# aras-p/ToyPathTracer

Measured on AMD Instinct MI355X. Metric: Mray/s, higher is better.
Workload: dtype f32

## Files before the change

toypathtracer_amd/csrc/tpt_device.h:

```cpp
#pragma once
#include "tpt_trace.h"

#ifndef TPT_BLOCK
#define TPT_BLOCK 64
#endif
#define TPT_CHUNK_PIXELS 256

namespace tpt {

struct KernelArgs {
    SceneView scene;
    FrameConsts fc;
    f4* frameColour;
    int nLocalRows, stripeRows, stripeStride, stripeOffset;
    int tilesX;
    int numItems;
    int numChunks, chunkSize;
    int batchFrames, chunksPerFrame, framePlane;
    unsigned totalWaves;
    int laneCap;
    int noRefill;
    f4* stackBuf;
    int stackStride;
    int ldsStackLevels;
    f4* pathBuf;
    const unsigned* chunkOrder;
    unsigned* chunkCost;
    int chunkShift;
    unsigned* work;
    unsigned long long* rayCounter;
    int rayCounterStride;
    unsigned gen;
    int helperBase;
    int helperPct;
    int ldsGroupPairs;
    const CameraPOD* viewCams = nullptr;
    const f4* moveCentres = nullptr;
    f4* aovSums = nullptr;
    f4* aovAlbedo = nullptr;
    f4* aovNormalDepth = nullptr;
    f4* momentsOut = nullptr;
    int aovPlane = 0;
    const int32_t* sampleCounts = nullptr;
    const f4* keyCentres = nullptr;
    unsigned long long keyMask = 0;
    int keyCount = 0;
};

}

hipError_t tptLaunchTrace(const tpt::KernelArgs& a, int hs, int fold, bool ldsScene, int blocks, size_t lds, hipStream_t stream);
int tptTraceOccupancy(int hs, int fold, bool ldsScene, size_t lds);
hipError_t tptLaunchTraceQueue(const tpt::KernelArgs& a, bool ldsScene, int blocks, size_t lds, hipStream_t stream);
int tptQueueMatrixFilter();
int tptQueueGroupMatrixBounds();
hipError_t tptLaunchDisplay(const float* tile, unsigned char* rgba, int width, int height, hipStream_t stream);
__attribute__((weak)) hipError_t tptLaunchDenoise(const float* colour, const float* albedo, const float* normalDepth, float* out,
                                                  float* scratch, int width, int height, int iterations, float ic, float in, float id,
                                                  bool demodulate, hipStream_t stream);
__attribute__((weak)) hipError_t tptLaunchDenoiseVariance(const float* colour, const float* albedo, const float* normalDepth,
                                                          const float* moments, float* out, float* scratch, int width, int height,
                                                          int iterations, float samples, float sl2, float in, float id, bool demodulate,
                                                          hipStream_t stream);
__attribute__((weak)) hipError_t tptLaunchFramesAtrous(const float* colour, const float* albedo, const float* normalDepth,
                                                       const float* moments, float* out, float* scratch, int width, int height, int frames,
                                                       int iterations, float samples, float sl2, float in, float id, bool demodulate,
                                                       hipStream_t stream);
struct tptTemporalConsts {
    float o[3], ll[3], H[3], V[3];
    float po[3], pa[3], pw[3], pH[3], pV[3];
    float pf, phh, pvv;
    float maxHistory, depthTol, normalTol, coverageTol;
};
__attribute__((weak)) hipError_t tptLaunchTemporal(const float* colour, const float* albedo, const float* normalDepth, const float* moments,
                                                   const float* prevColour, const float* prevAlbedo, const float* prevNormalDepth,
                                                   const float* prevMoments, float* outColour, float* outAlbedo, float* outMoments,
                                                   float* outVariance, int width, int height, const tptTemporalConsts& k,
                                                   hipStream_t stream);
struct tptObjectPlaneConsts {
// ... 53 lines not shown
```

toypathtracer_amd/csrc/tpt_host_pipeline.cpp:

```cpp
#include "tpt_context.h"

using namespace tpt;
using namespace tpth;

namespace tpth {

struct FramePlan {
    KernelArgs a;
    bool rowSerial = false, queued = false, ldsScene = false, useOrder = false;
    size_t lds = 0;
    int occ = 0, threadsPerBlock = 0, blocks = 0;
    int nOverlap = 1;
    int nSlots = 1, slot = 0;
    int batch = 1;
    bool plainFrame = true;
    const char* entry = "tptDrawDevice";
};

int syncAllStreams();
int reserveSlotBuffers(int nSlots, size_t colourBytes, size_t stackBytes)
{
    const bool small = colourBytes * 4 <= g.colourCap && g.colourCap * (size_t)g.slotsReserved > (1ull << 30);
    g.smallStreak = small ? g.smallStreak + 1 : 0;
    const bool shrink = small && g.smallStreak >= 8 && g.pending.empty();
// ... 504 lines not shown
            }
            (void)hipGetLastError();
        }
        HIPCHK(hipStreamWaitEvent(ts, g.evResolve[slot], 0));
    }
    if ((rc = enqueueSceneUpload(ts))) return rc;
    if (aov && ts != g.stream) {
        if (clip) {
            const unsigned h = g.clipSeq & 1u;
            HIPCHK(hipEventRecord(g.evClip[h ^ 1u], g.stream));
            HIPCHK(hipStreamWaitEvent(ts, aov->continues ? g.evClip[h] : g.evClip[h ^ 1u], 0));
        } else {
            HIPCHK(hipEventRecord(g.evAov, g.stream));
            HIPCHK(hipStreamWaitEvent(ts, g.evAov, 0));
        }
    }
    if (clip) g.clipSeq++;
    if (viewCams || centres || keyCentres) {
        static_assert(2 * sizeof(f4) * kMaxBatch <= sizeof(CameraPOD) * kMaxBatch, "a batch's moving centres fit the slot's camera table");
        Context::ViewSlot& V = g.views[slot];
        const f4* behind = keyCentres ? keyCentres : centres;
        const size_t camBytes = sizeof(CameraPOD) * (size_t)batch, centreBytes = (keyCentres ? (size_t)TPT_Q_KEYS_MAX : 2) * sizeof(f4) * (size_t)batch;
        const size_t bytes = viewCams && behind ? kViewCamBytes + centreBytes : (viewCams ? camBytes : centreBytes);
        if (V.copyEnqueued) HIPCHK(hipEventSynchronize(V.evUploaded));
        if (viewCams) memcpy(V.stage, viewCams, camBytes);
        if (behind) memcpy(reinterpret_cast<char*>(V.stage) + (viewCams ? kViewCamBytes : 0), behind, centreBytes);
        HIPCHK(hipMemcpyAsync(V.dev, V.stage, bytes, hipMemcpyHostToDevice, ts));
        HIPCHK(hipEventRecord(V.evUploaded, ts));
        V.copyEnqueued = true;
    }
    if ((rc = enqueueChunkOrder(P, ts))) return rc;
    if (frameRays && frameRays != g.dRays) HIPCHK(hipMemsetAsync(frameRays, 0, sizeof(unsigned long long) * (size_t)(rayStride > 0 ? batch : 1), ts));
    const bool helpable = P.queued && pipelined && batch == 1 && !P.rowSerial && !table && !aov;
    a.helperBase = 0;
    a.helperPct = 0;
    a.gen = 0u;
    g.hrec[slot].valid = false;
    if (helpable) {
        if (++g.launchGen == 0u) g.launchGen = 1u;
        a.gen = g.launchGen;
        HIPCHK(hipEventRecord(g.evPre[slot], ts));
    }
    const bool timeIt = g.kernelTiming && g.ktUsed < g.ktStart.size();
    if (timeIt) HIPCHK(hipEventRecord(g.ktStart[g.ktUsed], ts));
    if (P.queued)
        HIPCHK(tptLaunchTraceQueue(a, P.ldsScene, P.blocks, P.lds, ts));
    else
        HIPCHK(tptLaunchTrace(a, g.hs, g.foldMode, P.ldsScene, P.blocks, P.lds, ts));
    seqGuard.launched = true;
    if (timeIt) {
        HIPCHK(hipEventRecord(g.ktStop[g.ktUsed], ts));
        g.ktUsed++;
    }
    if (pipelined) HIPCHK(hipEventRecord(g.evTrace[slot], ts));
    if (helpable) {
        Context::HelperRec& R = g.hrec[slot];
        R.a = a; R.ldsScene = P.ldsScene; R.blocks = P.blocks; R.maxBlocks = maxGridBlocks(P); R.lds = P.lds;
        R.helped = false; R.valid = true; R.ts = ts;
    }
    T.slot = slot;
    T.nPixels = a.nLocalRows * w;
    T.pipelined = pipelined;
    T.lerpFac = a.fc.lerpFac;
    T.colour = a.frameColour;
    T.moments = a.momentsOut;
    T.batch = batch;
// ... 617 lines not shown
```

toypathtracer_amd/csrc/tpt_kernels.hip:

```cpp
#include "../../include/tpt_hip.h"
#include "tpt_device.h"
#include "tpt_queue_layout.h"
#include "tpt_shard.h"

namespace tpt {

__device__ __forceinline__ unsigned waveReduceAdd(unsigned v)
{
#pragma unroll
    for (int off = 32; off > 0; off >>= 1) v += __shfl_down(v, off, 64);
    return v;
}

__device__ __forceinline__ void storeColour(const KernelArgs& a, const Lane& L)
{
    f3 c = lanePixelColour(L, a.fc);
    f4 v;
    v.x = c.x; v.y = c.y; v.z = c.z; v.w = 0.0f;
    a.frameColour[L.pix] = v;
}

__global__ void __launch_bounds__(256) tptResolveKernel(float* __restrict__ tile, const f4* __restrict__ colour, int nPixels, float lerpFac,
                                                        const unsigned long long* frameRays, unsigned long long* totalRays)
{
// ... 1501 lines not shown
                    cm2 &= sel == 2 ? keep : ~0ull;
                    cm3 &= sel == 3 ? keep : ~0ull;
                    list[pos] = ((unsigned)p << 16) | (unsigned)((pb0 + sel * 32) * 2 + k);
                    ++pos;
                }
                if (!parked) {
                    st[p] = mk4(u2f((uint32_t)id), hitT, o.x, o.y);
                    st[PATHS + p] = mk4(o.z, d.x, d.y, d.z);
                    parked = true;
                }
            }
            __builtin_amdgcn_wave_barrier();
            dealProcessList<PATHS>(sv, list, listCount, st, lane);
            __builtin_amdgcn_wave_barrier();
        }
    }
    if (parked) {
        const f4 k = st[p];
        id = (int)f2u(k.x);
        hitT = k.y;
    }
    outT = hitT;
    return id;
}
#endif

#ifndef TPT_Q_MIN_WAVES_PER_SIMD
#define TPT_Q_MIN_WAVES_PER_SIMD 4
#endif
#ifndef TPT_Q_MAX_VGPR
#define TPT_Q_MAX_VGPR 60
#endif
template <bool LDS_SCENE, bool BATCH, bool VIEWS = false, bool MOVING = false, bool AOV = false, bool MOMENTS = false, bool ADAPTIVE = false,
          bool CAMERAS = false, bool KEYS = false>
__device__ __forceinline__ void traceQueueBody(const KernelArgs& a)
{
    extern __shared__ __attribute__((aligned(16))) unsigned char smem[];
    static_assert(BATCH || !VIEWS, "views are frames of a batched launch");
    static_assert((BATCH || !MOVING) && !(VIEWS && MOVING), "animation frames are frames of a batched launch of their own");
    static_assert(!AOV || !BATCH || (MOVING && MOMENTS), "first-hit planes are made by single-frame launches, or beside the moments of an animated clip's frames");
    static_assert(!MOMENTS || AOV, "moments are summed beside the first-hit sums");
    static_assert(!ADAPTIVE || (MOMENTS && !BATCH), "a count per pixel belongs to a single frame with its moments");
    static_assert(!CAMERAS || (BATCH && MOVING && AOV && MOMENTS && !VIEWS && !ADAPTIVE), "a camera per frame belongs to the frames of a clip with their planes");
    static_assert(!KEYS || CAMERAS, "the caller's centres per frame belong to the frames of a clip with their cameras and planes");
    constexpr bool CAM_TABLE = VIEWS || CAMERAS;
    constexpr int kMovedPerFrame = KEYS ? TPT_Q_KEYS_MAX : 2;
    constexpr int kPaths = (LDS_SCENE ? TPT_Q_PATHS : TPT_Q_PATHS_GROUPED) - (CAM_TABLE ? TPT_Q_VIEW_PATHS : 0) -
                           (MOVING ? (KEYS ? TPT_Q_KEY_PATHS : TPT_Q_ANIM_PATHS) : 0);
    constexpr int kOffSt = LDS_SCENE ? TPT_Q_SPH_FIXED : 0;
    constexpr int kOffQ = kOffSt + TPT_Q_NF4 * kPaths * 16;
    constexpr int kOffCtl = kOffQ + Q_COUNT * TPT_Q_P * 2;
    constexpr int kOffDeal = kOffCtl + (((int)sizeof(QueueCtl) + 63) & ~63);
    constexpr int kDealBytes = (!LDS_SCENE && TPT_GROUP_DEAL) ? TPT_Q_WAVES * TPT_GROUP_DEAL_WAVE_BYTES : 0;
    constexpr int kOffFc = kOffDeal + kDealBytes;
    constexpr int kOffCams = kOffFc + (((int)sizeof(FrameConsts) + 15) & ~15);
    constexpr int kOffMoved = kOffCams + (CAM_TABLE ? TPT_Q_VIEW_CAM_BYTES : 0);
    constexpr int kOffScene = kOffMoved + (MOVING ? (KEYS ? TPT_Q_KEY_TABLE_BYTES : TPT_Q_ANIM_TABLE_BYTES) : 0);
    f4* st = reinterpret_cast<f4*>(smem + kOffSt);
    LdsRing q = (LdsRing)(smem + kOffQ);
    QueueCtl* ctl = reinterpret_cast<QueueCtl*>(smem + kOffCtl);
    FrameConsts* ldsFc = reinterpret_cast<FrameConsts*>(smem + kOffFc);
    CameraPOD* ldsCams = reinterpret_cast<CameraPOD*>(smem + kOffCams);
    f4* ldsMoved = reinterpret_cast<f4*>(smem + kOffMoved);
    const LdsMovedPtr movedLds = (LdsMovedPtr)ldsMoved;
    const int nPad = a.scene.nPairs * 2;
    const bool sphFixed = LDS_SCENE && nPad * 16 <= TPT_Q_SPH_FIXED;
    f4* ldsSphFixed = reinterpret_cast<f4*>(smem);
    f4* ldsSph = sphFixed ? ldsSphFixed : reinterpret_cast<f4*>(smem + kOffScene);
    int off = kOffScene + ((LDS_SCENE && !sphFixed) ? nPad * 16 : 0);
// ... 58 lines not shown
        for (int i = tid; i < a.batchFrames * (int)(sizeof(CameraPOD) / 4); i += TPT_Q_T)
            reinterpret_cast<uint32_t*>(ldsCams)[i] = reinterpret_cast<const uint32_t*>(a.viewCams)[i];
    if (MOVING)
        for (int i = tid; i < a.batchFrames * kMovedPerFrame; i += TPT_Q_T) ldsMoved[i] = KEYS ? a.keyCentres[i] : a.moveCentres[i];
    const uint64_t keyMask = KEYS ? (uint64_t)a.keyMask : 0ull;
    for (int i = tid; i < Q_COUNT * TPT_Q_P; i += TPT_Q_T) q[i] = (unsigned short)(i < kPaths ? i : 0xFFFF);
    if (tid < 8) {
        ctl->head[tid] = 0u;
        ctl->tail[tid] = tid == Q_FREE ? (unsigned)kPaths : 0u;
    }
    if (tid == 0) {
        ctl->poolTotal = 0u;
        ctl->globalExhausted = 0u;
    }
    if (BATCH && tid < 32) ctl->frameRays[tid] = 0u;
    __syncthreads();

    const FrameConsts& fc = a.fc;
    const unsigned long long laneBelow = (1ull << lane) - 1ull;
#if TPT_MATRIX_FILTER
    SceneView svM = sv;
    svM.sph4 = ldsSphFixed;
#endif
#if TPT_GROUP_DEAL
    LdsList dealList = (LdsList)(smem + kOffDeal + (tid >> 6) * TPT_GROUP_DEAL_WAVE_BYTES);
    unsigned* dealCount = reinterpret_cast<unsigned*>(smem + kOffDeal + (tid >> 6) * TPT_GROUP_DEAL_WAVE_BYTES + TPT_GROUP_DEAL_ENTRIES * 4);
    const bool groupDeal = !MOVING && !LDS_SCENE && sv.nGroups > 0 && sv.nGroups <= 65536;
#endif
    f4* colSum = st + 2 * kPaths;
    int chunkNext = 0, chunkEnd = 0;
    int chunkFrame = 0;
    bool noMoreChunks = false;
    unsigned myRays = 0;
#if defined(TPT_STATS)
    const unsigned long long qT0 = wall_clock64();
    unsigned qSteps = 0, qBatches = 0, qIdle = 0;
    unsigned long long qSec[5] = {0, 0, 0, 0, 0};
#endif

#if defined(TPT_STATS)
#define TPT_TSTAMP(v)                      \
    __builtin_amdgcn_sched_barrier(0);     \
    __builtin_amdgcn_s_waitcnt(0);         \
    const unsigned long long v = __builtin_amdgcn_s_memtime(); \
    __builtin_amdgcn_sched_barrier(0)
#if TPT_STATS < 2
#define TPT_TADD(slot, a, b) do { if (lane == 0) atomicAdd(&g_tptStats[slot], (b) - (a)); } while (0)
#else
#define TPT_TADD(slot, a, b) do { qSec[(slot) == 64 + 24 ? 4 : ((slot) & 3)] += (b) - (a); } while (0)
#endif
#else
#define TPT_TSTAMP(v) do { } while (0)
#define TPT_TADD(slot, a, b) do { } while (0)
#endif
    for (;;) {
        TPT_TSTAMP(tsTop);
        unsigned myAvail = 0, myHead = 0, myTail = 0;
        if (lane < Q_COUNT) {
            myTail = __hip_atomic_load(&ctl->tail[lane], __ATOMIC_RELAXED, __HIP_MEMORY_SCOPE_WORKGROUP);
            myHead = __hip_atomic_load(&ctl->head[lane], __ATOMIC_RELAXED, __HIP_MEMORY_SCOPE_WORKGROUP);
            myAvail = myTail - myHead;
        }
        unsigned avail[Q_COUNT];
#pragma unroll
        for (int c = 0; c < Q_COUNT; ++c) avail[c] = (unsigned)__builtin_amdgcn_readlane((int)myAvail, c);
        const bool canStart = (chunkEnd > chunkNext) || !noMoreChunks;
// ... 55 lines not shown
        QStack stack;
        stack.l0 = (LdsF4Ptr)(st + 3 * kPaths + p);
        stack.spill = a.stackBuf + ((size_t)(blockIdx.x + (unsigned)a.helperBase) * TPT_Q_PATHS + p);
        stack.stride = a.stackStride;
        constexpr int kAovSums = MOMENTS ? 3 : 2;
        auto aovSum = [&]() { return a.aovSums + kAovSums * ((size_t)(blockIdx.x + (unsigned)a.helperBase) * TPT_Q_PATHS + p); };
        QLambert lam;
        lam.sdir = lam.nl = lam.albedo = lam.lightE = mk3(0, 0, 0);
        lam.cosAMax = 0.0f;
        int movedAt = 0;
        if (pick != Q_FREE && mine) {
            if (MOVING) movedAt = kMovedPerFrame * (int)(f2u(colSum[p].w) >> 26);
            const f4 r0 = st[0 * kPaths + p], r1 = st[1 * kPaths + p];
            ro = mk3(r0.x, r0.y, r0.z);
            rng = f2u(r0.w);
            rd = mk3(r1.x, r1.y, r1.z);
            const uint32_t w = f2u(r1.w);
            sample = (int)(w & 0x7ffu);
            depth = (int)((w >> 11) & 15u);
            doMatE = ((w >> 15) & 1u) != 0;
            recId = (w >> 16) == 0xffffu ? -1 : (int)(w >> 16);
        }

        if (pick == Q_FREE) {
            bool need = mine, got = false;
            int px = 0, py = 0, laneFrame = 0;
            [[maybe_unused]] uint32_t laneCount = 0u;
            for (;;) {
                const unsigned long long needMask = __ballot(need);
                if (needMask == 0ull) break;
                if (chunkNext >= chunkEnd) {
                    if (noMoreChunks) break;
                    int c = 0;
                    if (lane == 0) {
                        atomicAdd(&ctl->poolTotal, 64u);
                        c = (int)atomicAdd(&a.work[0], 1u);
                    }
                    c = __builtin_amdgcn_readfirstlane(c);
                    if (c >= a.numChunks) {
                        if (lane == 0) {
                            atomicSub(&ctl->poolTotal, 64u);
                            __hip_atomic_store(&ctl->globalExhausted, 1u, __ATOMIC_RELAXED, __HIP_MEMORY_SCOPE_WORKGROUP);
                        }
                        noMoreChunks = true;
                        break;
                    }
                    chunkFrame = 0;
                    if (BATCH) {
                        chunkFrame = c / a.chunksPerFrame;
                        c -= chunkFrame * a.chunksPerFrame;
                    }
                    chunkNext = c * a.chunkSize;
                    chunkEnd = chunkNext + a.chunkSize;
                    if (chunkEnd > a.numItems) chunkEnd = a.numItems;
                    if (lane == 0 && chunkEnd - chunkNext != 64) atomicSub(&ctl->poolTotal, (unsigned)(64 - (chunkEnd - chunkNext)));
                }
                const int rank = __popcll(needMask & laneBelow);
                const int want = __popcll(needMask);
                const int availPx = chunkEnd - chunkNext;
                const int take = want < availPx ? want : availPx;
                if (need && rank < take) {
                    int x, ly;
                    bool take1 = mapItem(a, chunkNext + rank, x, ly);
                    if (ADAPTIVE && take1) {
                        const int c = a.sampleCounts[(size_t)ly * fc.width + x];
                        laneCount = (uint32_t)(c < 0 ? 0 : (c > 2047 ? 2047 : c));
                        take1 = laneCount != 0u;
                    }
                    if (take1) {
                        px = x;
                        py = localRowToGlobal(a, ly);
                        laneFrame = chunkFrame;
                        got = true;
                        need = false;
                    }
                }
                chunkNext += take;
                if (lane == 0) atomicSub(&ctl->poolTotal, (unsigned)take);
            }
            if (got) {
                rng = pixelSeed(fc.seedMode, px, py, fc.frame + ((BATCH && !VIEWS) ? laneFrame : 0));
// ... 120 lines not shown
                        const f4 l0 = MOVING ? movedOrKeyedSphere<KEYS>(sv.lights[j * 2], lightId, movedLds + movedAt, keyMask) : sv.lights[j * 2];
                        d2 = qLightRay(l0, ro, rng, lam.cosAMax, (sv.flags & SCENE_LIGHT_R2_DIV_SAFE) != 0);
                    }
                }
#if TPT_MATRIX_FILTER
                uint64_t cand = 0ull;
                if (LDS_SCENE && useMatrix) cand = phase1MatrixH(ldsA, mxR1, sv.nSpheres, ro, d2);
#endif
#if TPT_GROUP_DEAL
                int dealId = -1;
                float dealT = TPT_MAX_T;
                if (!LDS_SCENE && groupDeal)
                    dealId = hitSpheresGroupedDeal<kPaths>(sv, go, ro, d2, dealT, dealList, dealCount, st, p, lane, ldsGpairs, a.ldsGroupPairs);
#endif
                if (go) {
                    TPT_STAT(ST_STEP);
                    float t;
                    int id;
#if TPT_GROUP_DEAL
                    if (!LDS_SCENE && groupDeal) {
                        id = dealId;
                        t = dealT;
                    } else
#endif
#if TPT_MATRIX_FILTER
                    if (LDS_SCENE && useMatrix)
                        id = hitSpheresCandidates<MOVING, KEYS>(svM, cand, ro, d2, TPT_MIN_T, TPT_MAX_T, t, movedLds + movedAt, keyMask);
                    else
#endif
                    if (MOVING)
                        id = hitSpheresTwoPhase<true, KEYS>(sv, ro, d2, TPT_MIN_T, TPT_MAX_T, t, movedLds + movedAt, keyMask);
                    else
                        id = hitSpheres<LDS_SCENE ? HS_TWO_PHASE : HS_TWO_PHASE_GROUPS>(sv, ro, d2, TPT_MIN_T, TPT_MAX_T, t);
                    if (BATCH) iterRays++; else myRays++;
                    if (shadow) {
                        if (id == lightId) qLightShade(l1, d2, lam);
                    } else {
                        hitId = id;
                        hitT = t;
                    }
                }
            }
            if (ray) {
                if (hitId < 0 || depth >= TPT_MAX_DEPTH)
                    cls = Q_END;
                else {
                    const int type = (int)f2u(sv.mats[hitId * 3].w);
                    cls = type == MAT_LAMBERT ? Q_LAMBERT : type == MAT_METAL ? Q_METAL : type == MAT_DIELECTRIC ? Q_DIEL : Q_END;
                }
                if (hitId >= 0) ro = ro + rd * hitT;
                if (AOV && depth == 0 && hitId >= 0) {
                    const f3 nrm = qNormal<MOVING, KEYS>(sv, hitId, ro, movedLds + movedAt, keyMask);
                    const f4 m0 = sv.mats[hitId * 3];
                    f4* sum = aovSum();
                    const f4 s0 = sum[0], s1 = sum[1];
                    sum[0] = mk4(s0.x + m0.x, s0.y + m0.y, s0.z + m0.z, s0.w + 1.0f);
                    sum[1] = mk4(s1.x + nrm.x, s1.y + nrm.y, s1.z + nrm.z, s1.w + hitT);
                }
                recId = hitId;
            }
        } else if (ray) {
            cls = Q_INT;
        }
        if (toEnd) cls = Q_END;
        if (ray || toEnd) {
            const uint32_t w = ((uint32_t)sample & 0x7ffu) | (((uint32_t)depth & 15u) << 11) | ((uint32_t)doMatE << 15) | (((uint32_t)recId & 0xffffu) << 16);
            st[0 * kPaths + p] = mk4(ro.x, ro.y, ro.z, u2f(rng));
            st[1 * kPaths + p] = mk4(rd.x, rd.y, rd.z, u2f(w));
        }
        if (toFree) cls = Q_FREE;
        if (BATCH && iterRays != 0u) {
            const unsigned fr = f2u(colSum[p].w) >> 26;
            const unsigned old = atomicAdd(&ctl->frameRays[fr], iterRays);
            if (__builtin_expect(old < 0x80000000u && old + iterRays >= 0x80000000u, 0)) {
                atomicSub(&ctl->frameRays[fr], 0x80000000u);
                atomicAdd(a.rayCounter + (size_t)fr * a.rayCounterStride, 0x80000000ull);
            }
        }
        TPT_TSTAMP(tsInt);
        TPT_TADD(64 + pick * 4 + 2, tsClass, tsInt);
        __builtin_amdgcn_fence(__ATOMIC_RELEASE, "workgroup");
        qPushByClass(q, ctl, mine ? cls : -1, p, lane);
        TPT_TSTAMP(tsPush);
        TPT_TADD(64 + pick * 4 + 3, tsInt, tsPush);
    }

    const unsigned waveRays = waveReduceAdd(myRays);
    if (BATCH) {
        __syncthreads();
        if (tid < a.batchFrames && ctl->frameRays[tid] != 0u) atomicAdd(a.rayCounter + (size_t)tid * a.rayCounterStride, (unsigned long long)ctl->frameRays[tid]);
    }
    if (helper) {
        if (lane == 0 && !BATCH) atomicAdd(a.rayCounter, (unsigned long long)waveRays);
        __syncthreads();
        if (tid == 0) {
            __builtin_amdgcn_fence(__ATOMIC_RELEASE, "agent");
            __hip_atomic_fetch_sub(&a.work[2], 1u, __ATOMIC_SEQ_CST, __HIP_MEMORY_SCOPE_AGENT);
        }
        return;
    }
    if (lane == 0) {
        if (!BATCH) atomicAdd(a.rayCounter, (unsigned long long)waveRays);
        unsigned done = atomicAdd(&a.work[1], 1u) + 1u;
        if (done == a.totalWaves) {
            if (a.gen != 0u) {
                const unsigned prev = __hip_atomic_exchange(&a.work[3], a.gen, __ATOMIC_RELAXED, __HIP_MEMORY_SCOPE_AGENT);
                unsigned busy = __hip_atomic_fetch_or(&a.work[2], dependentZero(prev), __ATOMIC_RELAXED, __HIP_MEMORY_SCOPE_AGENT);
                while (busy != 0u) {
                    __builtin_amdgcn_s_sleep(127);
                    busy = __hip_atomic_fetch_or(&a.work[2], 0u, __ATOMIC_RELAXED, __HIP_MEMORY_SCOPE_AGENT);
                }
            }
            a.work[0] = 0u;
            a.work[1] = 0u;
        }
    }
#if defined(__HIP_DEVICE_COMPILE__) && defined(TPT_STATS) && TPT_STATS >= 2
    __syncthreads();
    if (tid < 4) TPT_COUNT(120 + tid, g_hsLds[tid]);
#if TPT_GROUP_DEAL
    if (tid < 15) TPT_COUNT(90 + tid, g_dealLds[tid]);
    if (tid >= 15 && tid < 18) TPT_COUNT(124 + tid - 15, g_dealLds[tid]);
#endif
#endif
#if defined(TPT_STATS)
    if (lane == 0) {
        const unsigned long long qT1 = wall_clock64();
        TPT_COUNT(106, qSteps);
        TPT_COUNT(107, waveRays);
        TPT_COUNT(108, qT1 - qT0);
        TPT_COUNT(109, 1);
        TPT_COUNT(110, qBatches);
        TPT_COUNT(105, qIdle);
#if TPT_STATS >= 2
        for (int k = 0; k < 5; ++k) TPT_COUNT(112 + k, qSec[k]);
#endif
    }
#endif
}

#ifndef TPT_Q_MAX_VGPR_GROUPED
#define TPT_Q_MAX_VGPR_GROUPED 64
#endif
template <bool LDS_SCENE, bool BATCH = false>
__global__ void __launch_bounds__(TPT_Q_T, TPT_Q_MIN_WAVES_PER_SIMD) __attribute__((amdgpu_num_vgpr(TPT_Q_MAX_VGPR)))
tptTraceQueueKernel(const KernelArgs a)
{
    traceQueueBody<LDS_SCENE, BATCH>(a);
}
template <>
__global__ void __launch_bounds__(TPT_Q_T, TPT_Q_MIN_WAVES_PER_SIMD) __attribute__((amdgpu_num_vgpr(TPT_Q_MAX_VGPR_GROUPED)))
tptTraceQueueKernel<false, false>(const KernelArgs a)
{
    traceQueueBody<false, false>(a);
}
template <>
__global__ void __launch_bounds__(TPT_Q_T, TPT_Q_MIN_WAVES_PER_SIMD) __attribute__((amdgpu_num_vgpr(TPT_Q_MAX_VGPR_GROUPED)))
tptTraceQueueKernel<false, true>(const KernelArgs a)
{
    traceQueueBody<false, true>(a);
}
enum { QF_BATCH = 1, QF_VIEWS = 2, QF_MOVING = 4, QF_AOV = 8, QF_MOMENTS = 16, QF_ADAPTIVE = 32, QF_CAMERAS = 64, QF_KEYS = 128 };
#define TPT_QUEUE_VARIANT_KERNEL(NAME, F)                                                                                                    \
    template <bool LDS_SCENE>                                                                                                                \
    __global__ void __launch_bounds__(TPT_Q_T, TPT_Q_MIN_WAVES_PER_SIMD) __attribute__((amdgpu_num_vgpr(TPT_Q_MAX_VGPR)))                    \
    NAME(const KernelArgs a)                                                                                                                 \
    {                                                                                                                                        \
        traceQueueBody<LDS_SCENE, ((F) & QF_BATCH) != 0, ((F) & QF_VIEWS) != 0, ((F) & QF_MOVING) != 0, ((F) & QF_AOV) != 0, ((F) & QF_MOMENTS) != 0, \
                       ((F) & QF_ADAPTIVE) != 0, ((F) & QF_CAMERAS) != 0, ((F) & QF_KEYS) != 0>(a);                                                             \
    }                                                                                                                                        \
    template <>                                                                                                                              \
    __global__ void __launch_bounds__(TPT_Q_T, TPT_Q_MIN_WAVES_PER_SIMD) __attribute__((amdgpu_num_vgpr(TPT_Q_MAX_VGPR_GROUPED)))            \
    NAME<false>(const KernelArgs a)                                                                                                          \
    {                                                                                                                                        \
        traceQueueBody<false, ((F) & QF_BATCH) != 0, ((F) & QF_VIEWS) != 0, ((F) & QF_MOVING) != 0, ((F) & QF_AOV) != 0, ((F) & QF_MOMENTS) != 0, \
                       ((F) & QF_ADAPTIVE) != 0, ((F) & QF_CAMERAS) != 0, ((F) & QF_KEYS) != 0>(a);                                                             \
    }
TPT_QUEUE_VARIANT_KERNEL(tptTraceViewsKernel, QF_BATCH | QF_VIEWS)
TPT_QUEUE_VARIANT_KERNEL(tptTraceAnimationKernel, QF_BATCH | QF_MOVING)
TPT_QUEUE_VARIANT_KERNEL(tptTraceAovKernel, QF_AOV)
TPT_QUEUE_VARIANT_KERNEL(tptTraceMomentsKernel, QF_AOV | QF_MOMENTS)
TPT_QUEUE_VARIANT_KERNEL(tptTraceClipKernel, QF_BATCH | QF_MOVING | QF_AOV | QF_MOMENTS)
TPT_QUEUE_VARIANT_KERNEL(tptTraceAdaptiveKernel, QF_AOV | QF_MOMENTS | QF_ADAPTIVE)
TPT_QUEUE_VARIANT_KERNEL(tptCameraClipKernel, QF_BATCH | QF_MOVING | QF_AOV | QF_MOMENTS | QF_CAMERAS)
TPT_QUEUE_VARIANT_KERNEL(tptKeyframeKernel, QF_BATCH | QF_MOVING | QF_AOV | QF_MOMENTS | QF_CAMERAS | QF_KEYS)
#undef TPT_QUEUE_VARIANT_KERNEL

#if defined(TPT_TEST_HOOKS)
__global__ void tptMathTestKernel(int op, const float* __restrict__ a, const float* __restrict__ b, float* __restrict__ out, int n)
{
    int i = blockIdx.x * blockDim.x + threadIdx.x;
    if (i >= n) return;
    float x = a[i], y = b ? b[i] : 0.0f, r = 0.0f;
    switch (op) {
    case 0: r = tsqrt(x); break;
    case 1: r = x / y; break;
    case 2: r = tsinf(x); break;
    case 3: r = tcosf(x); break;
    case 4: r = tpow5f(x); break;
    case 5: {
        uint32_t s = f2u(x) | 1u;
        for (int k = 0; k < 16; ++k) r = rnd01(s);
        break;
    }
    case 6: r = schlick(x, y); break;
    case 7: r = normalize(mk3(x, y, 1.0f)).x; break;
    case 8: { float sn, cs; tsincosf(x, sn, cs); r = sn; break; }
    case 9: { float sn, cs; tsincosf(x, sn, cs); r = cs; break; }
    case 10: r = tdivSafeNum(x, y); break;
    case 11: r = tdivByPi(x); break;
    }
    out[i] = r;
}

__global__ void __launch_bounds__(256) tptMathExhaustiveKernel(int op, uint32_t lo, uint32_t hi, unsigned long long* nBad, uint32_t* firstBad)
{
    const uint64_t n = (uint64_t)hi - lo + 1;
    for (uint64_t i = (uint64_t)blockIdx.x * blockDim.x + threadIdx.x; i < n; i += (uint64_t)gridDim.x * blockDim.x) {
// ... 185 lines not shown
        case 6: return FN<HS_SIMPLE, FOLD_FORWARD, false>(__VA_ARGS__);                        \
        default: return FN<HS_SIMPLE, FOLD_FORWARD, true>(__VA_ARGS__);                        \
        }                                                                                      \
    } while (0)

hipError_t tptLaunchTrace(const KernelArgs& a, int hs, int fold, bool ldsScene, int blocks, size_t lds, hipStream_t stream)
{
    TPT_DISPATCH(launchOne, a, blocks, lds, stream);
}
int tptTraceOccupancy(int hs, int fold, bool ldsScene, size_t lds)
{
    TPT_DISPATCH(occupancyOne, lds);
}

static hipError_t launchQueueKernel(void (*k)(KernelArgs), const KernelArgs& a, int blocks, size_t lds, hipStream_t stream)
{
    hipError_t e = hipFuncSetAttribute(reinterpret_cast<const void*>(k), hipFuncAttributeMaxDynamicSharedMemorySize, (int)lds);
    if (e != hipSuccess) return e;
    hipLaunchKernelGGL(k, dim3(blocks), dim3(TPT_Q_T), lds, stream, a);
    return hipGetLastError();
}
hipError_t tptLaunchTraceQueue(const KernelArgs& a, bool ldsScene, int blocks, size_t lds, hipStream_t stream)
{
    static void (*const kernel[QV_INVALID][2])(KernelArgs) = {
         {tptTraceQueueKernel<false, false>, tptTraceQueueKernel<true, false>},
         {tptTraceQueueKernel<false, true>, tptTraceQueueKernel<true, true>},
         {tptTraceViewsKernel<false>, tptTraceViewsKernel<true>},
         {tptTraceAnimationKernel<false>, tptTraceAnimationKernel<true>},
         {tptTraceAovKernel<false>, tptTraceAovKernel<true>},
         {tptTraceMomentsKernel<false>, tptTraceMomentsKernel<true>},
         {tptTraceClipKernel<false>, tptTraceClipKernel<true>},
         {tptTraceAdaptiveKernel<false>, tptTraceAdaptiveKernel<true>},
         {tptKeyframeKernel<false>, tptKeyframeKernel<true>},
         {tptCameraClipKernel<false>, tptCameraClipKernel<true>},
    };
    const QueueVariant variant = tptQueueVariant(a);
    if (variant == QV_INVALID) return hipErrorInvalidValue;
    return launchQueueKernel(kernel[variant][ldsScene ? 1 : 0], a, blocks, lds, stream);
}
#if defined(TPT_TEST_HOOKS)
hipError_t tptSetDealCapacitiesForTest(int ca, int cb, int cs)
{
    unsigned v[3] = {TPT_DEAL_CA, TPT_DEAL_CB, TPT_DEAL_CS};
    if (ca || cb || cs) {
        if (ca < 64 || ca > TPT_DEAL_CA || cb < 64 || cb > TPT_DEAL_CB || cs < 64 || cs > TPT_DEAL_CS) return hipErrorInvalidValue;
        v[0] = (unsigned)ca; v[1] = (unsigned)cb; v[2] = (unsigned)cs;
    }
    return hipMemcpyToSymbol(HIP_SYMBOL(g_dealCaps), v, sizeof(v));
}
#endif
int tptQueueMatrixFilter() { return TPT_MATRIX_FILTER; }
int tptQueueGroupMatrixBounds() { return TPT_MATRIX_FILTER && TPT_GROUP_MATRIX_BOUNDS; }

hipError_t tptLaunchDisplay(const float* tile, unsigned char* rgba, int width, int height, hipStream_t stream)
{
    hipLaunchKernelGGL(tptDisplayKernel, dim3((width * height + 255) / 256), dim3(256), 0, stream, reinterpret_cast<const f4*>(tile),
                       reinterpret_cast<uint32_t*>(rgba), width, height);
    return hipGetLastError();
}

template <typename Launch>
static hipError_t atrousIterations(const float* colour, float* out, float* scratch, int iterations, Launch launch)
{
    const f4* src = reinterpret_cast<const f4*>(colour);
    for (int i = 0; i < iterations; ++i) {
        f4* dst = reinterpret_cast<f4*>(((iterations - 1 - i) & 1) ? scratch : out);
        launch(i, src, dst);
        hipError_t e = hipGetLastError();
        if (e != hipSuccess) return e;
        src = dst;
// ... 238 lines not shown
```

toypathtracer_amd/csrc/tpt_queue_layout.h:

```cpp
#pragma once
#include "tpt_device.h"
#include "tpt_shard.h"

#ifndef TPT_Q_WAVES
#define TPT_Q_WAVES 8
#endif
#define TPT_Q_T (64 * TPT_Q_WAVES)
#ifndef TPT_Q_P
#define TPT_Q_P 1024
#endif
#ifndef TPT_MATRIX_FILTER
#define TPT_MATRIX_FILTER 1
#endif
#ifndef TPT_GROUP_DEAL
#define TPT_GROUP_DEAL 1
#endif
#ifndef TPT_GROUP_MATRIX_BOUNDS
#if defined(TPT_TEST_HOOKS)
#define TPT_GROUP_MATRIX_BOUNDS 1
#else
#define TPT_GROUP_MATRIX_BOUNDS 0
#endif
#endif
#ifndef TPT_GROUP_DEAL_EXACT
// ... 56 lines not shown
static_assert(sizeof(QueueCtl::frameRays) / 4 == TPT_Q_VIEWS_MAX, "one ray count per frame of a batch");
static_assert(sizeof(tptLerpTable::v) / sizeof(float) == TPT_Q_VIEWS_MAX, "one lerp factor per frame of a batch");
static_assert(TPT_Q_VIEWS_MAX <= 64, "the path record holds 6 bits of frame index");

constexpr size_t kQueueLdsFixedPart = (size_t)TPT_Q_NF4 * TPT_Q_PATHS * 16 + (size_t)Q_COUNT * TPT_Q_P * 2 + ((sizeof(tpt::QueueCtl) + 63) & ~(size_t)63) +
                                      ((sizeof(tpt::FrameConsts) + 15) & ~(size_t)15);
constexpr size_t kDefaultSceneLds = TPT_Q_SPH_FIXED + ((46 * 4 + 15) & ~15) + 46 * 48 + 2 * 32 + (TPT_MATRIX_FILTER ? TPT_MXH_TABLE_DWORDS * 4 + 64 : 0);
static_assert(2 * (kQueueLdsFixedPart + kDefaultSceneLds + 256) <= 160 * 1024, "the default scene no longer fits two path-queue workgroups per CU: shrink TPT_Q_PATHS");
static_assert(TPT_Q_VIEW_CAM_BYTES <= TPT_Q_NF4 * TPT_Q_VIEW_PATHS * 16, "the views' cameras take no more LDS than the path records they replace");
static_assert(sizeof(tpt::CameraPOD) == 88 && sizeof(tpt::CameraPOD) % 4 == 0, "cameras are staged in LDS as 22 words");
static_assert(TPT_Q_ANIM_TABLE_BYTES == TPT_Q_NF4 * TPT_Q_ANIM_PATHS * 16, "the moving centres take exactly the LDS of the path records they replace");
static_assert(TPT_Q_KEY_TABLE_BYTES == TPT_Q_NF4 * TPT_Q_KEY_PATHS * 16 && TPT_Q_KEY_PATHS == 64, "the keyed centres take exactly the LDS of the 64 path records they replace");
static_assert(TPT_Q_KEYS_MAX <= 64 && TPT_Q_VIEW_PATHS + TPT_Q_KEY_PATHS < TPT_Q_PATHS_GROUPED, "a keyed sphere's slot is a popcount of the 64-bit mask; path records are left");

TPT_HD bool mapItem(const KernelArgs& a, int idx, int& x, int& ly)
{
    if (a.fc.seedMode == SEED_ROW_SERIAL) {
        x = 0;
        ly = idx;
        return ly < a.nLocalRows;
    }
    int tile = idx >> 6, within = idx & 63;
    const int tilesX = uniformHere(a.tilesX);
    int tx = tile % tilesX, ty = tile / tilesX;
    x = tx * 8 + (within & 7);
    ly = ty * 8 + (within >> 3);
    return x < a.fc.width && ly < a.nLocalRows;
}
TPT_HD int localRowToGlobal(const KernelArgs& a, int ly) { return shardKernelLocalToGlobal(ly, uniformHere(a.stripeRows), uniformHere(a.stripeStride), a.stripeOffset); }
TPT_HD int globalRowToLocal(const KernelArgs& a, int gy) { return shardKernelGlobalToLocal(gy, uniformHere(a.stripeRows), uniformHere(a.stripeStride), a.stripeOffset); }

}

enum QueueVariant { QV_FRAME, QV_BATCH, QV_VIEWS, QV_ANIMATION, QV_AOV, QV_MOMENTS, QV_CLIP, QV_ADAPTIVE, QV_KEYFRAME_CLIP, QV_CAMERA_CLIP, QV_INVALID };
inline QueueVariant tptQueueVariant(const tpt::KernelArgs& a)
{
    if (a.keyCentres) {
        if (a.batchFrames < 1 || a.batchFrames > TPT_Q_VIEWS_MAX || a.scene.nGroups > 0 || !a.viewCams || a.moveCentres || a.sampleCounts || !a.aovSums ||
            !a.momentsOut || a.keyCount < 0 || a.keyCount > TPT_Q_KEYS_MAX)
            return QV_INVALID;
        return QV_KEYFRAME_CLIP;
    }
    if (a.sampleCounts) {
        if (a.batchFrames != 1 || a.viewCams || a.moveCentres || !a.aovSums || !a.momentsOut) return QV_INVALID;
        return QV_ADAPTIVE;
    }
    if (a.viewCams && a.moveCentres) {
        if (a.batchFrames < 1 || a.batchFrames > TPT_Q_VIEWS_MAX || a.scene.nGroups > 0 || !a.aovSums || !a.momentsOut) return QV_INVALID;
        return QV_CAMERA_CLIP;
    }
    if (a.viewCams) {
        if (a.batchFrames < 1 || a.batchFrames > TPT_Q_VIEWS_MAX) return QV_INVALID;
        return QV_VIEWS;
    }
    if (a.aovSums && a.moveCentres) {
        if (a.batchFrames < 1 || a.batchFrames > TPT_Q_VIEWS_MAX || a.scene.nGroups > 0 || !a.momentsOut) return QV_INVALID;
        return QV_CLIP;
    }
    if (a.aovSums) {
        if (a.batchFrames != 1 || a.viewCams || a.moveCentres) return QV_INVALID;
        return a.momentsOut ? QV_MOMENTS : QV_AOV;
    }
    if (a.moveCentres) {
        if (a.batchFrames < 1 || a.batchFrames > TPT_Q_VIEWS_MAX || a.scene.nGroups > 0) return QV_INVALID;
        return QV_ANIMATION;
    }
    return a.batchFrames > 1 ? QV_BATCH : QV_FRAME;
}

// ... 40 lines not shown
```

Before: 45320.

## Give each frame of a batched launch its own block pool and chunk counter

Adds a frame-pools queue kernel variant in which each block is statically assigned to one frame of a batch, drawing chunks from a per-frame atomic counter instead of one global counter. Ray counting then goes per wave straight to the frame's counter, skipping the per-path frame-ray LDS atomics and the end-of-block flush. This is meant to reduce contention on the single work counter and the per-frame ray bookkeeping. The cost is the loss of dynamic load balancing across frames, since a pool whose frame finishes early cannot help the others, and it only applies to plain batched launches with enough blocks.

```diff
diff --git a/toypathtracer_amd/csrc/tpt_device.h b/toypathtracer_amd/csrc/tpt_device.h
--- a/toypathtracer_amd/csrc/tpt_device.h
+++ b/toypathtracer_amd/csrc/tpt_device.h
@@ -1,5 +1,6 @@
 #pragma once
 #include "tpt_trace.h"
+#include "tpt_frame_pools.h"
 
 #ifndef TPT_BLOCK
 #define TPT_BLOCK 64
@@ -45,6 +46,7 @@
     const f4* keyCentres = nullptr;
     unsigned long long keyMask = 0;
     int keyCount = 0;
+    int framePools = 0;
 };
 
 }
diff --git a/toypathtracer_amd/csrc/tpt_frame_pools.h b/toypathtracer_amd/csrc/tpt_frame_pools.h
--- /dev/null
+++ b/toypathtracer_amd/csrc/tpt_frame_pools.h
@@ -0,0 +1,24 @@
+#pragma once
+
+#if defined(__HIPCC__)
+#define TPT_FP_HD __host__ __device__ inline
+#else
+#define TPT_FP_HD inline
+#endif
+
+namespace tpt {
+
+const int kFramePoolBase = 4;
+const int kFramePoolsMax = 8;
+
+TPT_FP_HD int framePoolsOfLaunch(int batch, int blocks, bool plain, bool helpable)
+{
+    return (plain && !helpable && batch >= 2 && batch <= kFramePoolsMax && blocks >= 2 * batch) ? batch : 0;
+}
+
+TPT_FP_HD unsigned framePoolOfBlock(unsigned block, unsigned pools, unsigned blocks)
+{
+    return block * pools / blocks;
+}
+
+}
diff --git a/toypathtracer_amd/csrc/tpt_host_pipeline.cpp b/toypathtracer_amd/csrc/tpt_host_pipeline.cpp
--- a/toypathtracer_amd/csrc/tpt_host_pipeline.cpp
+++ b/toypathtracer_amd/csrc/tpt_host_pipeline.cpp
@@ -560,6 +560,7 @@
     if ((rc = enqueueChunkOrder(P, ts))) return rc;
     if (frameRays && frameRays != g.dRays) HIPCHK(hipMemsetAsync(frameRays, 0, sizeof(unsigned long long) * (size_t)(rayStride > 0 ? batch : 1), ts));
     const bool helpable = P.queued && pipelined && batch == 1 && !P.rowSerial && !table && !aov;
+    a.framePools = framePoolsOfLaunch(batch, P.blocks, P.queued && !P.rowSerial && !table && !aov, helpable);
     a.helperBase = 0;
     a.helperPct = 0;
     a.gen = 0u;
diff --git a/toypathtracer_amd/csrc/tpt_kernels.hip b/toypathtracer_amd/csrc/tpt_kernels.hip
--- a/toypathtracer_amd/csrc/tpt_kernels.hip
+++ b/toypathtracer_amd/csrc/tpt_kernels.hip
@@ -1557,9 +1557,10 @@
 #define TPT_Q_MAX_VGPR 60
 #endif
 template <bool LDS_SCENE, bool BATCH, bool VIEWS = false, bool MOVING = false, bool AOV = false, bool MOMENTS = false, bool ADAPTIVE = false,
-          bool CAMERAS = false, bool KEYS = false>
+          bool CAMERAS = false, bool KEYS = false, bool POOLS = false>
 __device__ __forceinline__ void traceQueueBody(const KernelArgs& a)
 {
+    static_assert(!POOLS || (BATCH && !VIEWS && !MOVING && !AOV), "a pool per frame belongs to the plain batched launch");
     extern __shared__ __attribute__((aligned(16))) unsigned char smem[];
     static_assert(BATCH || !VIEWS, "views are frames of a batched launch");
     static_assert((BATCH || !MOVING) && !(VIEWS && MOVING), "animation frames are frames of a batched launch of their own");
@@ -1684,6 +1685,7 @@
     int chunkFrame = 0;
     bool noMoreChunks = false;
     unsigned myRays = 0;
+    auto poolFrame = [&]() { return framePoolOfBlock(blockIdx.x, (unsigned)uniformHere(a.batchFrames), (unsigned)uniformHere((int)gridDim.x)); };
 #if defined(TPT_STATS)
     const unsigned long long qT0 = wall_clock64();
     unsigned qSteps = 0, qBatches = 0, qIdle = 0;
@@ -1805,12 +1807,13 @@
                 if (chunkNext >= chunkEnd) {
                     if (noMoreChunks) break;
                     int c = 0;
+                    [[maybe_unused]] const int myFrame = POOLS ? (int)poolFrame() : 0;
                     if (lane == 0) {
                         atomicAdd(&ctl->poolTotal, 64u);
-                        c = (int)atomicAdd(&a.work[0], 1u);
+                        c = (int)atomicAdd(POOLS ? &a.work[kFramePoolBase + myFrame] : &a.work[0], 1u);
                     }
                     c = __builtin_amdgcn_readfirstlane(c);
-                    if (c >= a.numChunks) {
+                    if (c >= (POOLS ? a.chunksPerFrame : a.numChunks)) {
                         if (lane == 0) {
                             atomicSub(&ctl->poolTotal, 64u);
                             __hip_atomic_store(&ctl->globalExhausted, 1u, __ATOMIC_RELAXED, __HIP_MEMORY_SCOPE_WORKGROUP);
@@ -1819,7 +1822,9 @@
                         break;
                     }
                     chunkFrame = 0;
-                    if (BATCH) {
+                    if (POOLS) {
+                        chunkFrame = myFrame;
+                    } else if (BATCH) {
                         chunkFrame = c / a.chunksPerFrame;
                         c -= chunkFrame * a.chunksPerFrame;
                     }
@@ -2006,7 +2011,7 @@
                         id = hitSpheresTwoPhase<true, KEYS>(sv, ro, d2, TPT_MIN_T, TPT_MAX_T, t, movedLds + movedAt, keyMask);
                     else
                         id = hitSpheres<LDS_SCENE ? HS_TWO_PHASE : HS_TWO_PHASE_GROUPS>(sv, ro, d2, TPT_MIN_T, TPT_MAX_T, t);
-                    if (BATCH) iterRays++; else myRays++;
+                    if (BATCH && !POOLS) iterRays++; else myRays++;
                     if (shadow) {
                         if (id == lightId) qLightShade(l1, d2, lam);
                     } else {
@@ -2043,7 +2048,7 @@
             st[1 * kPaths + p] = mk4(rd.x, rd.y, rd.z, u2f(w));
         }
         if (toFree) cls = Q_FREE;
-        if (BATCH && iterRays != 0u) {
+        if (BATCH && !POOLS && iterRays != 0u) {
             const unsigned fr = f2u(colSum[p].w) >> 26;
             const unsigned old = atomicAdd(&ctl->frameRays[fr], iterRays);
             if (__builtin_expect(old < 0x80000000u && old + iterRays >= 0x80000000u, 0)) {
@@ -2060,7 +2065,7 @@
     }
 
     const unsigned waveRays = waveReduceAdd(myRays);
-    if (BATCH) {
+    if (BATCH && !POOLS) {
         __syncthreads();
         if (tid < a.batchFrames && ctl->frameRays[tid] != 0u) atomicAdd(a.rayCounter + (size_t)tid * a.rayCounterStride, (unsigned long long)ctl->frameRays[tid]);
     }
@@ -2075,6 +2080,7 @@
     }
     if (lane == 0) {
         if (!BATCH) atomicAdd(a.rayCounter, (unsigned long long)waveRays);
+        if (POOLS) atomicAdd(a.rayCounter + (size_t)poolFrame() * a.rayCounterStride, (unsigned long long)waveRays);
         unsigned done = atomicAdd(&a.work[1], 1u) + 1u;
         if (done == a.totalWaves) {
             if (a.gen != 0u) {
@@ -2087,6 +2093,8 @@
             }
             a.work[0] = 0u;
             a.work[1] = 0u;
+            if (POOLS)
+                for (int j = 0; j < a.batchFrames; ++j) a.work[kFramePoolBase + j] = 0u;
         }
     }
 #if defined(__HIP_DEVICE_COMPILE__) && defined(TPT_STATS) && TPT_STATS >= 2
@@ -2134,21 +2142,21 @@
 {
     traceQueueBody<false, true>(a);
 }
-enum { QF_BATCH = 1, QF_VIEWS = 2, QF_MOVING = 4, QF_AOV = 8, QF_MOMENTS = 16, QF_ADAPTIVE = 32, QF_CAMERAS = 64, QF_KEYS = 128 };
+enum { QF_BATCH = 1, QF_VIEWS = 2, QF_MOVING = 4, QF_AOV = 8, QF_MOMENTS = 16, QF_ADAPTIVE = 32, QF_CAMERAS = 64, QF_KEYS = 128, QF_POOLS = 256 };
 #define TPT_QUEUE_VARIANT_KERNEL(NAME, F)                                                                                                    \
     template <bool LDS_SCENE>                                                                                                                \
     __global__ void __launch_bounds__(TPT_Q_T, TPT_Q_MIN_WAVES_PER_SIMD) __attribute__((amdgpu_num_vgpr(TPT_Q_MAX_VGPR)))                    \
     NAME(const KernelArgs a)                                                                                                                 \
     {                                                                                                                                        \
         traceQueueBody<LDS_SCENE, ((F) & QF_BATCH) != 0, ((F) & QF_VIEWS) != 0, ((F) & QF_MOVING) != 0, ((F) & QF_AOV) != 0, ((F) & QF_MOMENTS) != 0, \
-                       ((F) & QF_ADAPTIVE) != 0, ((F) & QF_CAMERAS) != 0, ((F) & QF_KEYS) != 0>(a);                                                             \
+                       ((F) & QF_ADAPTIVE) != 0, ((F) & QF_CAMERAS) != 0, ((F) & QF_KEYS) != 0, ((F) & QF_POOLS) != 0>(a);                                                            \
     }                                                                                                                                        \
     template <>                                                                                                                              \
     __global__ void __launch_bounds__(TPT_Q_T, TPT_Q_MIN_WAVES_PER_SIMD) __attribute__((amdgpu_num_vgpr(TPT_Q_MAX_VGPR_GROUPED)))            \
     NAME<false>(const KernelArgs a)                                                                                                          \
     {                                                                                                                                        \
         traceQueueBody<false, ((F) & QF_BATCH) != 0, ((F) & QF_VIEWS) != 0, ((F) & QF_MOVING) != 0, ((F) & QF_AOV) != 0, ((F) & QF_MOMENTS) != 0, \
-                       ((F) & QF_ADAPTIVE) != 0, ((F) & QF_CAMERAS) != 0, ((F) & QF_KEYS) != 0>(a);                                                             \
+                       ((F) & QF_ADAPTIVE) != 0, ((F) & QF_CAMERAS) != 0, ((F) & QF_KEYS) != 0, ((F) & QF_POOLS) != 0>(a);                                                            \
     }
 TPT_QUEUE_VARIANT_KERNEL(tptTraceViewsKernel, QF_BATCH | QF_VIEWS)
 TPT_QUEUE_VARIANT_KERNEL(tptTraceAnimationKernel, QF_BATCH | QF_MOVING)
@@ -2158,6 +2166,7 @@
 TPT_QUEUE_VARIANT_KERNEL(tptTraceAdaptiveKernel, QF_AOV | QF_MOMENTS | QF_ADAPTIVE)
 TPT_QUEUE_VARIANT_KERNEL(tptCameraClipKernel, QF_BATCH | QF_MOVING | QF_AOV | QF_MOMENTS | QF_CAMERAS)
 TPT_QUEUE_VARIANT_KERNEL(tptKeyframeKernel, QF_BATCH | QF_MOVING | QF_AOV | QF_MOMENTS | QF_CAMERAS | QF_KEYS)
+TPT_QUEUE_VARIANT_KERNEL(tptFramePoolsKernel, QF_BATCH | QF_POOLS)
 #undef TPT_QUEUE_VARIANT_KERNEL
 
 #if defined(TPT_TEST_HOOKS)
@@ -2409,10 +2418,12 @@
          {tptTraceClipKernel<false>, tptTraceClipKernel<true>},
          {tptTraceAdaptiveKernel<false>, tptTraceAdaptiveKernel<true>},
          {tptKeyframeKernel<false>, tptKeyframeKernel<true>},
+         {tptFramePoolsKernel<false>, tptFramePoolsKernel<true>},
          {tptCameraClipKernel<false>, tptCameraClipKernel<true>},
     };
     const QueueVariant variant = tptQueueVariant(a);
     if (variant == QV_INVALID) return hipErrorInvalidValue;
+    if (variant == QV_FRAME_POOLS && blocks < a.framePools) return hipErrorInvalidValue;
     return launchQueueKernel(kernel[variant][ldsScene ? 1 : 0], a, blocks, lds, stream);
 }
 #if defined(TPT_TEST_HOOKS)
diff --git a/toypathtracer_amd/csrc/tpt_queue_layout.h b/toypathtracer_amd/csrc/tpt_queue_layout.h
--- a/toypathtracer_amd/csrc/tpt_queue_layout.h
+++ b/toypathtracer_amd/csrc/tpt_queue_layout.h
@@ -112,9 +112,15 @@
 
 }
 
-enum QueueVariant { QV_FRAME, QV_BATCH, QV_VIEWS, QV_ANIMATION, QV_AOV, QV_MOMENTS, QV_CLIP, QV_ADAPTIVE, QV_KEYFRAME_CLIP, QV_CAMERA_CLIP, QV_INVALID };
+enum QueueVariant { QV_FRAME, QV_BATCH, QV_VIEWS, QV_ANIMATION, QV_AOV, QV_MOMENTS, QV_CLIP, QV_ADAPTIVE, QV_KEYFRAME_CLIP, QV_FRAME_POOLS, QV_CAMERA_CLIP, QV_INVALID };
 inline QueueVariant tptQueueVariant(const tpt::KernelArgs& a)
 {
+    if (a.framePools != 0) {
+        if (a.framePools != a.batchFrames || a.framePools < 2 || a.framePools > tpt::kFramePoolsMax || a.helperBase > 0 || a.viewCams || a.moveCentres ||
+            a.keyCentres || a.sampleCounts || a.aovSums || a.fc.seedMode == tpt::SEED_ROW_SERIAL)
+            return QV_INVALID;
+        return QV_FRAME_POOLS;
+    }
     if (a.keyCentres) {
         if (a.batchFrames < 1 || a.batchFrames > TPT_Q_VIEWS_MAX || a.scene.nGroups > 0 || !a.viewCams || a.moveCentres || a.sampleCounts || !a.aovSums ||
             !a.momentsOut || a.keyCount < 0 || a.keyCount > TPT_Q_KEYS_MAX)
```

Measured after the change: 46080, median of 6. 1.7% higher.
